# lazear/sage

Measured on AMD Instinct MI355X. Metric: spectra/sec (whole node), fragment-index search-and-score, human tryptic narrow search, higher is better.
Workload: dtype f32

## Files before the change

include/sage_hip.h:

```cpp
#ifndef SAGE_HIP_H
#define SAGE_HIP_H

#include <stddef.h>
#include <stdint.h>

#ifdef __cplusplus
extern "C" {
#endif

#define SAGE_HIP_ABI_VERSION 6

enum {
    SAGE_HIP_OK = 0,
    SAGE_HIP_ERR_INVALID = 1,
    SAGE_HIP_ERR_NO_DEVICE = 2,
    SAGE_HIP_ERR_HIP = 3,
    SAGE_HIP_ERR_UNSUPPORTED = 4,
    SAGE_HIP_ERR_OOM = 5,
    SAGE_HIP_ERR_INTERNAL = 6
};

enum { SAGE_TOL_PPM = 0, SAGE_TOL_PCT = 1, SAGE_TOL_DA = 2 };
typedef struct SageTolerance {
    int32_t kind;
// ... 161 lines not shown
    uint64_t* psm_off;
    uint8_t* kinds;
    int32_t* charges;
    int32_t* fragment_ordinals;
    float* intensities;
    float* mz_calculated;
    float* mz_experimental;
} SageFragments;
int sage_hip_annotate_resident(SageScorer* scorer, SageDeviceBatch* batch, const SageFeature* features,
                               const uint32_t* counts, SageFragments* out);

int sage_hip_quick_score_resident(SageScorer* scorer, SageDeviceBatch* batch, int prefilter_low_memory, uint8_t* keep);

typedef struct SageTiming {
    float prelim_ms;
    float rescore_ms;
    float total_ms;
    uint32_t n_launches;
    uint32_t n_wide;
    uint32_t arena_entries;
    uint32_t n_retry;
    float retry_ms;
    uint32_t n_tied;
    uint32_t n_ways;
} SageTiming;
int sage_hip_last_timing(const SageScorer* scorer, SageTiming* out);
int sage_hip_scorer_set_timing_interval(SageScorer* scorer, uint32_t every);

int sage_hip_host_alloc(uint64_t bytes, void** out);
void sage_hip_host_free(void* p);

int sage_hip_debug_phase_cycles(SageScorer* scorer, unsigned long long* out32);
int sage_hip_debug_prune_counters(SageScorer* scorer, unsigned long long* out4);

typedef struct SageRescoreInput {
    uint64_t n;
    const SageFeature* features;
    const float* aligned_rt;
    const float* delta_rt_model;
    const float* delta_ims_model;
    SageTolerance precursor_tol;
    const uint32_t* peptide_key;
    uint32_t n_peptide_keys;
    const uint32_t* protein_key;
    uint32_t n_protein_keys;
} SageRescoreInput;

typedef struct SageRescoreOutput {
    float* discriminant_score;
    float* posterior_error;
    float* spectrum_q;
    float* peptide_q;
    float* protein_q;
    uint32_t* order;
    uint64_t passing_spectrum;
    uint64_t passing_peptide;
    uint64_t passing_protein;
    int32_t lda_fitted;
    double coef[20];
    float device_ms;
} SageRescoreOutput;

int sage_hip_rescore(int device, const SageRescoreInput* in, SageRescoreOutput* out);

typedef struct SageRtInput {
    uint64_t n;
// ... 168 lines not shown
```

sage_amd/_lib.py:

```python
import ctypes as C
import os

import numpy as np

from . import build as _build

c_float_p = C.POINTER(C.c_float)
c_u8_p = C.POINTER(C.c_uint8)
c_u32_p = C.POINTER(C.c_uint32)
c_u64_p = C.POINTER(C.c_uint64)


class SageTolerance(C.Structure):
    _fields_ = [("kind", C.c_int32), ("lo", C.c_float), ("hi", C.c_float)]


class SageTheoretical(C.Structure):
    _fields_ = [("peptide_index", C.c_uint32), ("fragment_mz", C.c_float)]


class SageDbParams(C.Structure):
    _fields_ = [
        ("bucket_size", C.c_uint64),
        ("missed_cleavages", C.c_int32),
# ... 242 lines not shown
        "sage_hip_hostdb_build": (C.c_int, [C.c_char_p, C.POINTER(SageDbParams), C.POINTER(vp)]),
        "sage_hip_hostdb_free": (None, [vp]),
        "sage_hip_hostdb_view": (C.c_int, [vp, C.POINTER(SageDbView)]),
        "sage_hip_hostdb_peptide_string": (C.c_uint64, [vp, C.c_uint64, C.c_char_p, C.c_uint64]),
        "sage_hip_hostdb_peptide_proteins": (C.c_uint64, [vp, C.c_uint64, C.c_char_p, C.c_uint64]),
        "sage_hip_hostdb_peptide_info": (C.c_int, [vp, C.c_uint64, c_u32_p, c_u8_p]),
        "sage_hip_process_ms2": (C.c_uint64, [C.c_uint64, C.c_int, C.c_float, c_float_p, c_float_p, C.c_uint64,
                                              C.c_uint8, c_float_p, c_float_p, c_float_p]),
        "sage_hip_device_count": (C.c_int, []),
        "sage_hip_db_create": (C.c_int, [C.POINTER(SageDbView), C.c_int, C.POINTER(vp)]),
        "sage_hip_db_destroy": (None, [vp]),
        "sage_hip_db_device_bytes": (C.c_uint64, [vp]),
        "sage_hip_scorer_create": (C.c_int, [vp, C.POINTER(SageScorerParams), C.POINTER(vp)]),
        "sage_hip_scorer_destroy": (None, [vp]),
        "sage_hip_scorer_clone": (C.c_int, [vp, C.POINTER(vp)]),
        "sage_hip_score_batch": (C.c_int, [vp, C.POINTER(SageSpectrumBatch), vp, c_u32_p]),
        "sage_hip_batch_upload": (C.c_int, [vp, C.POINTER(SageSpectrumBatch), C.POINTER(vp)]),
        "sage_hip_batch_free": (None, [vp]),
        "sage_hip_batch_process_upload": (C.c_int, [vp, C.POINTER(SageRawBatch), C.c_uint64, C.c_int, C.c_float, C.c_uint32,
                                                    C.POINTER(vp), c_u32_p]),
        "sage_hip_batch_download": (C.c_int, [vp, c_u64_p, c_float_p, c_float_p, c_float_p]),
        "sage_hip_batch_upload_kinds": (C.c_int, [vp, C.POINTER(SageSpectrumBatch), c_u8_p, C.POINTER(vp)]),
        "sage_hip_batch_process_upload_kinds": (C.c_int, [vp, C.POINTER(SageRawBatch), c_u8_p, C.c_uint64, C.c_int, C.c_float,
                                                          C.c_uint32, C.POINTER(vp), c_u32_p]),
        "sage_hip_score_batch_kinds": (C.c_int, [vp, C.POINTER(SageSpectrumBatch), c_u8_p, vp, c_u32_p]),
        "sage_hip_score_resident": (C.c_int, [vp, vp, vp, c_u32_p]),
        "sage_hip_initial_hits": (C.c_int, [vp, vp, c_u64_p, C.c_uint32, c_u32_p, c_u64_p, c_u64_p]),
        "sage_hip_last_timing": (C.c_int, [vp, C.POINTER(SageTiming)]),
        "sage_hip_scorer_set_timing_interval": (C.c_int, [vp, C.c_uint32]),
        "sage_hip_annotate_resident": (C.c_int, [vp, vp, vp, c_u32_p, C.POINTER(SageFragments)]),
        "sage_hip_quick_score_resident": (C.c_int, [vp, vp, C.c_int, c_u8_p]),
        "sage_hip_debug_phase_cycles": (C.c_int, [vp, c_u64_p]),
        "sage_hip_debug_prune_counters": (C.c_int, [vp, c_u64_p]),
        "sage_hip_host_alloc": (C.c_int, [C.c_uint64, C.POINTER(vp)]),
        "sage_hip_host_free": (None, [vp]),
        "sage_hip_rescore": (C.c_int, [C.c_int, C.POINTER(SageRescoreInput), C.POINTER(SageRescoreOutput)]),
        "sage_hip_hostdb_competition_keys": (C.c_int, [vp, c_u32_p, C.c_uint64, c_u32_p, c_u32_p, c_u32_p, c_u32_p]),
        "sage_hip_predict_rt": (C.c_int, [C.c_int, C.POINTER(SageRtInput), C.POINTER(SageRtOutput)]),
        "sage_hip_hostdb_feature_peptides": (C.c_int, [vp, c_u32_p, C.c_uint64, c_u64_p, c_u8_p, c_float_p]),
        "sage_hip_mzml_read": (C.c_int, [C.c_char_p, C.c_uint32, C.c_int, C.POINTER(vp)]),
        "sage_hip_mzml_view": (C.c_int, [vp, C.POINTER(SageRawBatch)]),
        "sage_hip_mzml_check_searchable": (C.c_int, [vp]),
        "sage_hip_mzml_spectrum_id": (C.c_char_p, [vp, C.c_uint64]),
        "sage_hip_mzml_free": (None, [vp]),
        "sage_hip_mzml_read_sn": (C.c_int, [C.c_char_p, C.c_uint32, C.c_int, C.c_int, C.POINTER(vp)]),
        "sage_hip_mzml_ion_injection_time": (C.c_float, [vp, C.c_uint64]),
        "sage_hip_mzml_precursor_ref": (C.c_char_p, [vp, C.c_uint64]),
        "sage_hip_mgf_read": (C.c_int, [C.c_char_p, C.c_uint32, C.POINTER(vp)]),
        "sage_hip_mzml_isolation_kinds": (C.c_int, [vp, c_u8_p]),
        "sage_hip_mzml_charge_zero": (C.c_int, [vp, c_u8_p]),
        "sage_hip_parse_f32": (C.c_int, [C.c_char_p, C.c_uint64, c_float_p]),
        "sage_hip_tmt": (C.c_int, [C.c_int, C.POINTER(SageTmtInput), C.POINTER(SageTmtOutput)]),
        "sage_hip_write_tmt": (C.c_int, [C.c_char_p, C.POINTER(C.c_char_p), C.c_uint32, C.c_uint64, c_u32_p, C.POINTER(C.c_char_p),
                                         c_float_p, c_float_p, C.POINTER(C.c_char_p), C.c_uint32]),
        "sage_hip_write_results": (C.c_int, [C.c_char_p, C.c_int, vp, vp, C.c_uint64, c_u64_p, c_u64_p, C.POINTER(C.c_char_p),
                                             C.c_uint32, C.POINTER(C.c_char_p), C.POINTER(SagePostColumns)]),
        "sage_hip_lfq": (C.c_int, [C.c_int, C.POINTER(SageLfqInput), C.POINTER(SageLfqOutput)]),
        "sage_hip_lfq_im": (C.c_int, [C.c_int, C.POINTER(SageLfqInput), C.POINTER(SageLfqMobility), C.POINTER(SageLfqOutput)]),
        "sage_hip_mzml_mobility": (c_float_p, [vp]),
        "sage_hip_mzml_has_mobility": (C.c_int, [vp, c_u8_p]),
        "sage_hip_write_lfq": (C.c_int, [C.c_char_p, vp, C.POINTER(SageLfqOutput), c_u64_p, C.c_uint64, C.POINTER(C.c_char_p),
                                         C.c_uint32]),
        "sage_hip_fasta_num_targets": (C.c_int, [C.c_char_p, C.POINTER(SageDbParams), c_u64_p]),
        "sage_hip_prefilter_chunk_size": (C.c_int, [C.c_char_p, C.POINTER(SageDbParams), C.c_uint64, c_u64_p]),
        "sage_hip_hostdb_build_chunk": (C.c_int, [C.c_char_p, C.POINTER(SageDbParams), C.c_uint64, C.c_uint64, C.POINTER(vp)]),
        "sage_hip_hostdb_merge_kept": (C.c_int, [C.POINTER(vp), C.POINTER(c_u8_p), C.c_uint32, C.POINTER(SageDbParams),
                                                 C.POINTER(vp)]),
    }
    for name, (res, args) in sig.items():
        fn = getattr(lib, name)
        fn.restype = res
        fn.argtypes = args
    _lib = lib
    return lib


EXPORTED_SYMBOLS = [
    "sage_hip_last_error", "sage_hip_abi_version", "sage_hip_hostdb_build", "sage_hip_hostdb_free",
    "sage_hip_hostdb_view", "sage_hip_hostdb_peptide_string", "sage_hip_hostdb_peptide_proteins",
    "sage_hip_hostdb_peptide_info", "sage_hip_process_ms2", "sage_hip_device_count", "sage_hip_db_create", "sage_hip_db_destroy",
    "sage_hip_db_device_bytes", "sage_hip_scorer_create", "sage_hip_scorer_destroy", "sage_hip_scorer_clone", "sage_hip_score_batch",
    "sage_hip_batch_upload", "sage_hip_batch_free", "sage_hip_batch_process_upload", "sage_hip_batch_download", "sage_hip_score_resident", "sage_hip_initial_hits",
    "sage_hip_last_timing", "sage_hip_scorer_set_timing_interval", "sage_hip_annotate_resident", "sage_hip_quick_score_resident", "sage_hip_debug_phase_cycles", "sage_hip_debug_prune_counters", "sage_hip_host_alloc", "sage_hip_host_free",
    "sage_hip_rescore", "sage_hip_hostdb_competition_keys", "sage_hip_fasta_num_targets", "sage_hip_prefilter_chunk_size",
    "sage_hip_hostdb_build_chunk", "sage_hip_hostdb_merge_kept", "sage_hip_predict_rt", "sage_hip_hostdb_feature_peptides",
    "sage_hip_write_results", "sage_hip_mzml_read", "sage_hip_mzml_view", "sage_hip_mzml_check_searchable", "sage_hip_mzml_spectrum_id", "sage_hip_mzml_free",
    "sage_hip_lfq", "sage_hip_write_lfq", "sage_hip_mzml_read_sn", "sage_hip_mzml_ion_injection_time", "sage_hip_mzml_precursor_ref",
    "sage_hip_tmt", "sage_hip_write_tmt", "sage_hip_mgf_read", "sage_hip_mzml_isolation_kinds", "sage_hip_mzml_charge_zero",
    "sage_hip_parse_f32", "sage_hip_batch_upload_kinds", "sage_hip_batch_process_upload_kinds", "sage_hip_score_batch_kinds",
    "sage_hip_lfq_im", "sage_hip_mzml_mobility", "sage_hip_mzml_has_mobility",
]


def check(rc):
    if rc != 0:
        msg = load().sage_hip_last_error()
        raise SageHipError(f"libsage_hip status {rc}: {msg.decode() if msg else ''}")


def as_ptr(arr, ctype):
    return arr.ctypes.data_as(C.POINTER(ctype))
```

sage_amd/csrc/capi.hip:

```cpp
#include <hip/hip_runtime.h>
#include <algorithm>
#include <atomic>
#include <cmath>
#include <chrono>
#include <cstring>
#include <memory>
#include <future>
#include <mutex>
#include <string>
#include <vector>

#include "crlog.h"
#include "device_types.h"
#define HIP_FAILED(e, what) fail(status_of(e), std::string(what) + ": " + hipGetErrorString(e))
#include "hip_host.h"
#include "host_db.hpp"

using namespace sagehip;

namespace {

thread_local std::string g_last_error;

int fail(int code, const std::string& msg) {
// ... 2018 lines not shown
    if (rc != SAGE_HIP_OK) return rc;
    const uint32_t n = b->n, kmax = s->dev.kmax;
    std::vector<uint64_t> c((size_t)n * kmax);
    std::vector<uint32_t> tot((size_t)n * 2), st(n);
    HIP_TRY(hipMemcpy(c.data(), s->ws.cand.p, c.size() * 8, hipMemcpyDeviceToHost));
    HIP_TRY(hipMemcpy(len, s->ws.cand_len.p, (size_t)n * 4, hipMemcpyDeviceToHost));
    HIP_TRY(hipMemcpy(tot.data(), s->ws.totals.p, tot.size() * 4, hipMemcpyDeviceToHost));
    HIP_TRY(hipMemcpy(st.data(), s->ws.status.p, (size_t)n * 4, hipMemcpyDeviceToHost));
    for (uint32_t i = 0; i < n; i++) {
        if (st[i] != ST_OK && st[i] != ST_OK_ORDERED) return fail(SAGE_HIP_ERR_UNSUPPORTED, "spectrum " + std::to_string(i) + ": status " + std::to_string(st[i]));
        for (uint32_t j = 0; j < len[i]; j++) packed[(size_t)i * cap + j] = c[(size_t)i * kmax + j];
        if (matched_peaks) matched_peaks[i] = tot[2 * i];
        if (scored_candidates) scored_candidates[i] = tot[2 * i + 1];
    }
    return SAGE_HIP_OK;
}

int sage_hip_debug_phase_cycles(SageScorer* s, unsigned long long* out32) {
    if (!s || !out32) return fail(SAGE_HIP_ERR_INVALID, "null argument");
    if (!s->dbg.p) return fail(SAGE_HIP_ERR_INVALID, "set SAGE_HIP_PHASE_CLOCKS=1 before creating the scorer");
    std::vector<unsigned long long> all(4096 * 32);
    HIP_TRY(hipMemcpy(all.data(), s->dbg.p, all.size() * 8, hipMemcpyDeviceToHost));
    for (int k = 0; k < 32; k++) out32[k] = 0;
    for (size_t b = 0; b < 4096; b++)
        for (int k = 0; k < 32; k++) out32[k] += all[b * 32 + k];
    return SAGE_HIP_OK;
}

int sage_hip_debug_prune_counters(SageScorer* s, unsigned long long* out4) {
    if (!s || !out4) return fail(SAGE_HIP_ERR_INVALID, "null argument");
    if (!s->dbg.p) return fail(SAGE_HIP_ERR_INVALID, "set SAGE_HIP_PHASE_CLOCKS=1 before creating the scorer");
    std::vector<unsigned long long> all((size_t)DBG_BLOCKS * DBG_PRUNE_WORDS);
    HIP_TRY(hipMemcpy(all.data(), s->dbg.p + (size_t)DBG_BLOCKS * 32, all.size() * 8, hipMemcpyDeviceToHost));
    for (uint32_t k = 0; k < DBG_PRUNE_WORDS; k++) out4[k] = 0;
    for (size_t b = 0; b < DBG_BLOCKS; b++)
        for (uint32_t k = 0; k < DBG_PRUNE_WORDS; k++) out4[k] += all[b * DBG_PRUNE_WORDS + k];
    return SAGE_HIP_OK;
}

int sage_hip_host_alloc(uint64_t bytes, void** out) {
    if (!out) return fail(SAGE_HIP_ERR_INVALID, "null argument");
    HIP_TRY(hipHostMalloc(out, bytes ? bytes : 1, hipHostMallocDefault));
    if (void* d = device_view(*out)) {
        std::lock_guard<std::mutex> lock(g_blocks_mu);
        g_blocks.push_back(HostBlock{(const unsigned char*)*out, (unsigned char*)d, (size_t)(bytes ? bytes : 1)});
    }
    return SAGE_HIP_OK;
}
void sage_hip_host_free(void* p) {
    if (!p) return;
    {
        std::lock_guard<std::mutex> lock(g_blocks_mu);
        for (size_t i = 0; i < g_blocks.size(); i++)
            if (g_blocks[i].host == (const unsigned char*)p) {
                g_blocks.erase(g_blocks.begin() + (long)i);
                break;
            }
    }
    (void)hipHostFree(p);
}

int sage_hip_scorer_set_timing_interval(SageScorer* s, uint32_t every) {
    if (!s) return fail(SAGE_HIP_ERR_INVALID, "null argument");
    std::lock_guard<std::mutex> lock(s->mu);
    s->timing_every = every;
    s->timing_calls = 0;
    return SAGE_HIP_OK;
}

// ... 28 lines not shown
```

sage_amd/csrc/core.h:

```cpp
#pragma once
#include <stdint.h>

#if defined(__HIPCC__)
#define SAGE_HD __host__ __device__ __forceinline__
#else
#define SAGE_HD inline
#endif

namespace sagecore {

constexpr float PROTON = 1.0072764f;
constexpr float NEUTRON = 1.00335f;

struct Tol {
    int kind;
    float lo, hi;
};

SAGE_HD void tol_bounds(const Tol& t, float center, float& out_lo, float& out_hi) {
    if (t.kind == 0) {
        float dlo = center * t.lo / 1000000.0f;
        float dhi = center * t.hi / 1000000.0f;
        out_lo = center + dlo;
        out_hi = center + dhi;
// ... 477 lines not shown
    uint32_t x;
    asm("v_cvt_u32_f32 %0, %1" : "=v"(x) : "v"(f));
    return x;
#else
    const float f = ion * PBM_INV_W;
    return f >= 4294967296.0f ? 0xFFFFFFFFu : f > 0.0f ? (uint32_t)f : 0u;
#endif
}
SAGE_HD uint32_t pbm_bin_c1(uint32_t x) { return x & (PBM_BITS - 1u); }
SAGE_HD uint32_t pbm_bin_c2(uint32_t x) { return (x >> 1) & (PBM_BITS - 1u); }
SAGE_HD uint32_t pbm_bin_c3(uint32_t x) { return (uint32_t)(((uint64_t)x * 0xAAAAAAABull) >> 33) & (PBM_BITS - 1u); }
struct PbmReach {
    float a, b;
};
SAGE_HD PbmReach pbm_reach_of(const Tol& t) {
    const float tmax = __builtin_fmaxf(__builtin_fabsf(t.lo), __builtin_fabsf(t.hi));
    const float rel = t.kind == 0 ? tmax * 1.0e-6f : t.kind == 1 ? tmax * 1.0e-2f : 0.0f;
    PbmReach r{-1.0f, 0.0f};
    if (!(tmax == tmax) || !(tmax < 1.0e30f) || !(rel < 0.25f)) return r;
    r.a = (rel / (1.0f - rel)) * 1.0002f + (1.0f / 1048576.0f);
    r.b = (t.kind == 2 ? tmax * 1.0002f : 0.0f) + (1.0f / 1048576.0f);
    return r;
}
SAGE_HD bool pbm_peak_reach(const PbmReach& r, float m, float& D) {
    D = __builtin_fmaf(m, r.a, r.b);
    return r.a >= 0.0f && m >= 0.0f && m < 8388608.0f && D <= PBM_MAX_D;
}
SAGE_HD void pbm_peak_span(float m, float D, uint32_t& b0, uint32_t& b1) {
    const float f0 = (m - D) * PBM_INV_W, f1 = (m + D) * PBM_INV_W;
    b0 = f0 > 0.0f ? (uint32_t)f0 : 0u;
    b1 = f1 > 0.0f ? (uint32_t)f1 : 0u;
}

}
```

sage_amd/csrc/device_types.h:

```cpp
#pragma once
#include <stdint.h>

#include <string>

#include "../../include/sage_hip.h"
#include "core.h"

namespace sagehip {

struct DevDbView {
    const float* pep_mono;
    uint32_t np;
    const uint32_t* pep_lut;
    uint32_t pep_lut_bins;
    float pep_lut_inv_w;
    const SageTheoretical* pm_frag;
    const uint64_t* pm_off;
    const float* ions;
    const uint64_t* ion_off;
    const uint32_t* pep_info;
    const SageTheoretical* tm_frag;
    const uint32_t* tm_lut;
    uint32_t tile_shift;
    uint32_t n_tiles;
    uint32_t lut_stride;
    float lut_scale;
    const SageTheoretical* tm2_frag;
    const sagecore::LutWord* tm2_l1;
    const uint32_t* tm2_pos;
    uint32_t lut2_words;
    uint32_t tile2_shift;
    uint32_t n_tiles2;
    uint32_t lut2_stride;
    float lut2_scale;
    uint64_t nf;
    uint8_t ion_kinds[8];
    uint32_t n_kinds;
};

#ifndef SAGE_TM_LUT_TRANSPOSED
#define SAGE_TM_LUT_TRANSPOSED 0
#endif
#ifndef SAGE_TM_LUT_QUAD
#define SAGE_TM_LUT_QUAD 0
#endif
constexpr int TM_LUT_LAYOUT = SAGE_TM_LUT_QUAD != 0 ? 2 : SAGE_TM_LUT_TRANSPOSED != 0 ? 1 : 0;
constexpr bool TM_LUT_TRANSPOSED = TM_LUT_LAYOUT == 1;
__host__ __device__ inline uint32_t tm_lut_rows(uint32_t n_tiles) { return TM_LUT_LAYOUT == 2 ? (n_tiles + 3u) & ~3u : n_tiles; }
__host__ __device__ inline size_t tm_lut_index(uint32_t t, uint32_t c, uint32_t n_tiles, uint32_t lut_stride) {
    return TM_LUT_LAYOUT == 2 ? (((size_t)(t >> 2) * lut_stride + c) << 2) + (t & 3u)
           : TM_LUT_LAYOUT == 1 ? (size_t)c * n_tiles + t : (size_t)t * lut_stride + c;
}

constexpr uint32_t DBG_BLOCKS = 4096, DBG_PRUNE_WORDS = 4;
constexpr size_t DBG_TOTAL_WORDS = (size_t)DBG_BLOCKS * (32 + DBG_PRUNE_WORDS);

struct DevScorer {
    sagecore::Tol precursor_tol, fragment_tol;
    sagecore::PbmReach pbm_reach;
    uint32_t min_matched_peaks;
    int min_isotope_err, max_isotope_err;
    uint32_t min_precursor_charge, max_precursor_charge;
    uint32_t override_precursor_charge;
    int max_fragment_charge;
    uint32_t chimera;
    uint32_t report_psms;
    uint32_t wide_window;
    int score_type;
    uint32_t kmax;
    uint32_t big_path;
    uint32_t long_runs;
    uint32_t tol_mode;
    uint32_t list_cap;
    uint32_t wcap;
    uint32_t dbg_flags;
    uint32_t prune_min;
    uint32_t rescore_general;
    uint32_t xcd_chunk;
    uint32_t fast_log;
    uint32_t exact;
};

struct DevBatchView {
    uint32_t n;
    const uint32_t* n_dev;
    uint32_t spec_base;
    const uint64_t* peak_off;
// ... 160 lines not shown
```

sage_amd/csrc/kernels.hip:

```cpp
#include <hip/hip_runtime.h>

#include <type_traits>

#include "crlog.h"
#include "device_types.h"

using namespace sagecore;

namespace sagehip {

namespace {

constexpr uint32_t WAVE = 64;
constexpr uint32_t FAST_TIE_WORDS = PBM_WORDS + PLUT_BINS;
constexpr uint32_t CNT_ROW_HEADER = 4;
#ifndef SAGE_PROBE_PER_LANE
#define SAGE_PROBE_PER_LANE 2
#endif
constexpr uint32_t PROBE_BATCH_WORDS = SAGE_PROBE_PER_LANE * 64;
constexpr uint32_t PROBE_TCS_WORDS = PROBE_BATCH_WORDS <= 64 ? 64 : PROBE_BATCH_WORDS <= 128 ? 128 : PROBE_BATCH_WORDS <= 256 ? 256 : 512;
constexpr uint32_t PROBE_TABLE_WORDS = 4 * PROBE_BATCH_WORDS + PROBE_TCS_WORDS;

enum { DBG_PRUNE_CAND = 0, DBG_PRUNE_ITEMS = 1, DBG_PRUNE_EARLY = 2, DBG_PRUNE_MIXED = 3 };
enum { DBG_NARROW_LUT = 26, DBG_NARROW_CELLS = 27, DBG_RESCORE = 28, DBG_TILE_LUT = 29, DBG_TILE_CELLS = 30, DBG_TILE_CAND = 31 };
struct PhaseClock {
    unsigned long long* slot;
    long long t;
    __device__ __forceinline__ void bytes(int which, unsigned long long n) {
        if (slot) atomicAdd(&slot[which - row_base], n);
    }
    int row_base;
    unsigned long long* prune;
    uint32_t pruned_here;
    __device__ __forceinline__ void pruned(uint64_t lanes, uint32_t items) {
        if (slot && lanes) {
            pruned_here += (uint32_t)__popcll(lanes);
            if ((threadIdx.x & 63u) == 0) {
                atomicAdd(&prune[DBG_PRUNE_CAND], (unsigned long long)__popcll(lanes));
                atomicAdd(&prune[DBG_PRUNE_ITEMS], (unsigned long long)items);
            }
        }
    }
    __device__ __forceinline__ void prune_outcome(bool left_early, bool any_pass) {
        if (slot && (threadIdx.x & 63u) == 0) {
            if (left_early) atomicAdd(&prune[DBG_PRUNE_EARLY], 1ull);
            else if (any_pass && pruned_here) atomicAdd(&prune[DBG_PRUNE_MIXED], 1ull);
        }
        pruned_here = 0;
    }
    __device__ __forceinline__ void start(unsigned long long* dbg, uint32_t blk, uint32_t kernel) {
        slot = dbg ? dbg + (size_t)(blk % DBG_BLOCKS) * 32 + kernel * 8 : nullptr;
        row_base = (int)kernel * 8;
        prune = dbg ? dbg + (size_t)DBG_BLOCKS * 32 + (size_t)(blk % DBG_BLOCKS) * DBG_PRUNE_WORDS : nullptr;
        pruned_here = 0;
        if (slot) t = clock64();
    }
    __device__ __forceinline__ void mark(int phase) {
        if (slot) {
            const long long n = clock64();
            if ((threadIdx.x & 63u) == 0) atomicAdd(&slot[phase], (unsigned long long)(n - t));
            t = n;
        }
    }
    __device__ __forceinline__ void rebase(uint32_t kernel) {
        if (slot) slot += (int)kernel * 8 - row_base;
        row_base = (int)kernel * 8;
    }
};

struct NoClock {
    static constexpr unsigned long long* slot = nullptr;
    __device__ __forceinline__ void bytes(int, unsigned long long) {}
    __device__ __forceinline__ void pruned(uint64_t, uint32_t) {}
    __device__ __forceinline__ void prune_outcome(bool, bool) {}
    __device__ __forceinline__ void start(unsigned long long*, uint32_t, uint32_t) {}
    __device__ __forceinline__ void mark(int) {}
    __device__ __forceinline__ void rebase(uint32_t) {}
};

__device__ __forceinline__ uint32_t lane_id() { return threadIdx.x & 63u; }

#ifndef SAGE_STAGGER_NS
#define SAGE_STAGGER_NS 0
#endif
__device__ __forceinline__ void staggered_start(uint32_t blk) {
    if (SAGE_STAGGER_NS > 0 && blk >= 1024u && blk < 5u * 1024u) {
        const uint32_t slot = blk / 1024u;
        const long long until = (long long)__builtin_amdgcn_s_memtime() + (long long)slot * (SAGE_STAGGER_NS * 2);
        while ((long long)__builtin_amdgcn_s_memtime() < until) __builtin_amdgcn_s_sleep(32);
    }
}

constexpr uint32_t N_XCD = 8;
__device__ __forceinline__ uint32_t xcd_position_fwd(uint32_t b, uint32_t n, uint32_t chunk) {
    if (chunk == 0) return b;
    const uint32_t group = N_XCD * chunk;
    if (b >= n / group * group) return b;
    const uint32_t x = b % N_XCD, i = b / N_XCD;
    return ((i / chunk) * N_XCD + x) * chunk + i % chunk;
}
__device__ __forceinline__ uint32_t xcd_position(uint32_t b, uint32_t n, uint32_t chunk) {
    const uint32_t p = xcd_position_fwd(b, n, chunk & 0x7FFFFFFFu);
    return (chunk & 0x80000000u) ? n - 1 - p : p;
}

__device__ __forceinline__ uint32_t fresh_zero() {
    uint32_t z;
// ... 2442 lines not shown
    if (a.longest_b != b.longest_b) return a.longest_b > b.longest_b;
    if (a.longest_y != b.longest_y) return a.longest_y > b.longest_y;
    if (!(a.hyperscore == b.hyperscore)) return a.hyperscore > b.hyperscore;
    if (!(a.ppm_difference == b.ppm_difference)) return a.ppm_difference > b.ppm_difference;
    if (a.charge != b.charge) return a.charge > b.charge;
    return a.iso > b.iso;
}

struct RescoreLds {
    uint32_t* pbm;
    uint32_t* plut;
    double* s_sorted;
    long long* s_key;
    QuickKey* qkeys;
    uint32_t* hdr;
    uint2* meta;
    float* pm;
    float* pi;
    uint8_t* rm;
    uint8_t* rm2;
    uint32_t* stage;
};
constexpr uint32_t FEATURE_WORDS = sizeof(SageFeature) / 4;
static_assert(sizeof(SageFeature) == 120, "Feature records leave LDS as 30 dwords");
__host__ __device__ inline uint32_t stage_records(const DevScorer& sc) { return sc.big_path ? 0u : sc.chimera ? 1u : sc.report_psms; }
__host__ __device__ inline size_t rescore_scratch_bytes(bool quick) {
    static_assert(PBM_WORDS * 4 >= 64 * 8 + 64 * 8, "s_sorted + s_key fit the bitmap");
    static_assert(FAST_TIE_WORDS == PBM_WORDS + PLUT_BINS, "the fast-tie replay stages its counts over pbm + plut, contiguous below");
    return (size_t)PBM_WORDS * 4 + PLUT_BINS * 4 + (quick ? 64 * sizeof(QuickKey) : 0);
}
constexpr uint32_t RESCORE_HDR_WORDS = 8;
enum RescoreHdr { HDR_TIC = 0, HDR_MZP = 1, HDR_RT = 2, HDR_IMS = 3, HDR_FILE = 4, HDR_MATCHED = 5, HDR_SCORED = 6 };
constexpr size_t RESCORE_HEAD_BYTES = RESCORE_HDR_WORDS * 4 + 64 * sizeof(uint2);
__host__ __device__ inline size_t rescore_fixed_bytes(const DevScorer& sc, const DevBatchView& b) {
    const size_t n = RESCORE_HEAD_BYTES + (size_t)b.pcap * 8 + (((size_t)b.pcap * 2 + 7) & ~(size_t)7) + (size_t)stage_records(sc) * sizeof(SageFeature);
    return (n + 15) & ~(size_t)15;
}
__device__ __forceinline__ RescoreLds carve_rescore(unsigned char* scratch, unsigned char* fixed, const DevBatchView& b) {
    RescoreLds l;
    l.pbm = (uint32_t*)scratch;
    l.plut = l.pbm + PBM_WORDS;
    l.s_sorted = (double*)l.pbm;
    l.s_key = (long long*)(l.s_sorted + 64);
    l.qkeys = (QuickKey*)(l.plut + PLUT_BINS);
    l.hdr = (uint32_t*)fixed;
    l.meta = (uint2*)(fixed + RESCORE_HDR_WORDS * 4);
    l.pm = (float*)(fixed + RESCORE_HEAD_BYTES);
    l.pi = l.pm + b.pcap;
    l.rm = (uint8_t*)(l.pi + b.pcap);
    l.rm2 = l.rm + b.pcap;
    l.stage = (uint32_t*)(fixed + RESCORE_HEAD_BYTES + (size_t)b.pcap * 8 + (((size_t)b.pcap * 2 + 7) & ~(size_t)7));
    return l;
}

__device__ __forceinline__ uint32_t lane_run(uint32_t v, uint32_t src_lane) { return (uint32_t)__builtin_amdgcn_readlane((int)v, (int)src_lane); }
__device__ __forceinline__ uint64_t lane_run(uint64_t v, uint32_t src_lane) { return lane_value(v, src_lane); }
#ifndef SAGE_DENSE_HITS
#define SAGE_DENSE_HITS 1
#endif
constexpr uint32_t DENSE_CAP = 384;
static_assert(DENSE_CAP % 64 == 0 && DENSE_CAP * 10 + DENSE_CAP / 8 <= PBM_WORDS * 4, "the dense work list fits the bitmap");
template <class PC, bool LONG = false, bool FAST = false>
__device__ __forceinline__ void score_candidates(const DevDbView& db, const DevScorer& sc, const uint32_t* pbm, const uint32_t* plut,
                                                 const float* pm, const float* pi, const uint32_t P, const float inv_w,
                                                 const bool valid, const uint64_t ion_base, const uint32_t lm1, const uint32_t nfz,
                                                 const bool any_fz2, const bool any_fz3, const uint32_t nterm_mask, const bool sym_tol,
                                                 Score& s, PC& pc, const bool have_first = false, const float first0 = 0.f,
                                                 const float first1 = 0.f, const float first2 = 0.f, const float first3 = 0.f,
                                                 const bool dense_ok = false) {
    const uint32_t lane = lane_id();
    typedef typename std::conditional<LONG, uint64_t, uint32_t>::type RunReg;
    constexpr bool DENSE = !LONG;
    RunReg b_run = 0, y_run = 0;
    uint32_t mm = 0;
    const bool scored = valid && lm1 && nfz;
    const float* __restrict__ my = db.ions + ion_base;
    const uint32_t nions = scored ? db.n_kinds * lm1 : 0u;
    for (uint32_t j0 = 0; __ballot(j0 < nions) != 0ull; j0 += 64u) {
        const bool act = j0 < nions;
        const uint32_t n_here = !act ? 0u : nions - j0 < 64u ? nions - j0 : 64u;
        uint64_t m1 = 0, m2 = 0, m3 = 0;
        if (act) {
            const float* __restrict__ q = my + j0;
            float n0, n1, n2, n3;
            if (have_first && j0 == 0) { n0 = first0; n1 = first1; n2 = first2; n3 = first3; }
            else { n0 = q[0]; n1 = q[1]; n2 = q[2]; n3 = q[3]; }
            for (uint32_t r = 0; r < n_here; r += 4) {
                const float i0 = n0, i1 = n1, i2 = n2, i3 = n3;
                n0 = q[r + 4]; n1 = q[r + 5]; n2 = q[r + 6]; n3 = q[r + 7];
                const uint32_t x0 = pbm_index(i0), x1 = pbm_index(i1), x2 = pbm_index(i2), x3 = pbm_index(i3);
                const uint32_t t1 = pbm_bit(x0) | (pbm_bit(x1) << 1) | (pbm_bit(x2) << 2) | (pbm_bit(x3) << 3);
                m1 |= (uint64_t)t1 << r;
                if (any_fz2) {
                    const uint32_t t2 = pbm_bit(x0 >> 1) | (pbm_bit(x1 >> 1) << 1) | (pbm_bit(x2 >> 1) << 2) | (pbm_bit(x3 >> 1) << 3);
                    m2 |= (uint64_t)t2 << r;
                }
                if (any_fz3) {
                    const uint32_t t3 = pbm_bit(__umulhi(x0, 0xAAAAAAABu) >> 1) | (pbm_bit(__umulhi(x1, 0xAAAAAAABu) >> 1) << 1) |
                                        (pbm_bit(__umulhi(x2, 0xAAAAAAABu) >> 1) << 2) | (pbm_bit(__umulhi(x3, 0xAAAAAAABu) >> 1) << 3);
                    m3 |= (uint64_t)t3 << r;
                }
            }
            const uint64_t in_chunk = n_here >= 64u ? ~0ull : (1ull << n_here) - 1ull;
            m1 &= in_chunk;
            m2 = nfz >= 2 ? m2 & in_chunk : 0ull;
            m3 = nfz >= 3 ? m3 & in_chunk : 0ull;
            if (nfz > 3) m1 = m2 = m3 = in_chunk;
        }
        pc.mark(6);
        uint32_t hc = act && nfz <= 3 ? (uint32_t)(__popcll(m1) + __popcll(m2) + __popcll(m3)) : 0u;
        {
            const bool drop = hc != 0u && j0 + 64u >= nions && (mm & 0xFFFFu) + (mm >> 16) + hc < sc.prune_min;
            if (pc.slot) pc.pruned(__ballot(drop), wave_sum(drop ? hc : 0u));
            if (drop) {
                m1 = m2 = m3 = 0ull;
                hc = 0u;
            }
        }
        uint64_t bigs = (sc.dbg_flags & 32u) ? 0ull : __ballot(hc > COOP_MIN_HITS);
        if ((uint32_t)__popcll(bigs) > COOP_MAX_LANES && !(sc.dbg_flags & 64u)) bigs = 0ull;
        while (bigs) {
            const uint32_t L = (uint32_t)__ffsll((long long)bigs) - 1;
            bigs &= bigs - 1;
            const uint64_t M1 = lane_value(m1, L), M2 = lane_value(m2, L), M3 = lane_value(m3, L);
            const uint64_t base_L = lane_value((uint64_t)ion_base, L);
            const uint32_t lm1_L = (uint32_t)__builtin_amdgcn_readlane((int)lm1, (int)L);
            const bool on1 = (M1 >> lane) & 1ull, on2 = (M2 >> lane) & 1ull, on3 = (M3 >> lane) & 1ull;
            float it1 = 0.f, it2 = 0.f, it3 = 0.f, tm1 = 0.f, tm2 = 0.f, tm3 = 0.f;
            bool ok1 = false, ok2 = false, ok3 = false;
            if (on1 || on2 || on3) {
                const float ionv = db.ions[base_L + j0 + lane];
#define SAGE_COOP_LOOKUP(C, ON, OK, IT, TM)                                                              \
    if (ON) {                                                                                            \
        const float mz = fragment_mz<FAST>(ionv, (C));                                                   \
        float flo, fhi;                                                                                  \
// ... 333 lines not shown
        float first0 = 0.f, first1 = 0.f, first2 = 0.f, first3 = 0.f;
        if (round == 0 && valid) {
            const uint32_t plen = pep_rec & 0xFFFFu;
            lm1 = db.n_kinds && plen ? plen - 1u : 0u;
            R.meta[lane] = make_uint2(pep_rec, __float_as_uint(pep_mass));
            if (SAGE_ION_PREFETCH && lm1 && nfz) {
                const float* __restrict__ q = db.ions + ion_base;
                first0 = q[0]; first1 = q[1]; first2 = q[2]; first3 = q[3];
            }
        }
        if (round == 0) build_peak_bitmap(pbm, pm, P, sc.pbm_reach);
        lds_sync();
        if (round == 0) {
        if (pc.slot) {
            const uint32_t ion_bytes = wave_sum(valid ? 4u * db.n_kinds * lm1 + 24u : 0u);
            const uint32_t ncand = (uint32_t)__popcll(__ballot(mine != PRESCORE_EMPTY));
            if (lane == 0) pc.bytes(DBG_RESCORE, 8ull * P + 8ull * ncand + ion_bytes);
            const uint32_t items = wave_sum(SAGE_N_ITEMS);
            uint32_t longest = SAGE_N_ITEMS;
            for (int o = 32; o; o >>= 1) { const uint32_t v = (uint32_t)__shfl_xor((int)longest, o, 64); longest = v > longest ? v : longest; }
            const uint32_t nvalid = (uint32_t)__popcll(__ballot(valid));
            (void)items; (void)longest; (void)nvalid;
        }
        }
        Score s;
        s.peptide = 0;
        s.precursor_charge = 0;
        s.isotope_error = 0;
        s.matched_b = s.matched_y = 0;
        s.summed_b = s.summed_y = 0.0f;
        s.ppm_difference = 0.0f;
        s.longest_b = s.longest_y = 0;
        pc.mark(5);
        score_candidates<PC, false, FAST>(db, sc, pbm, plut, pm, pi, P, inv_w, valid, ion_base, lm1, nfz, any_fz2, any_fz3, nterm_mask, sym_tol,
                                          s, pc, SAGE_ION_PREFETCH && round == 0, first0, first1, first2, first3, !CHIMERA || !sc.chimera);
        pc.mark(1);
        LateArgs<KA> la(db, sc, b, w, lnfact_table, lnfact_n, out, out_count);
        la.refresh();
        {
            const uint32_t prune_min = la.prune_min();
            const uint64_t can_pass = __ballot(valid && s.matched_b + s.matched_y >= prune_min);
            const bool leave = prune_min != 0u && can_pass == 0ull;
            pc.prune_outcome(leave, can_pass != 0ull);
            if (leave) {
                if (ACC && keep) return true;
                break;
            }
        }
        const double lambda = (double)R.hdr[HDR_MATCHED] / (double)R.hdr[HDR_SCORED];
        double h = 0.0;
        bool pass = false;
        bool ln_undecided;
        const double ln_i = cr_log_pair<ACC>(hyperscore_arg(s), lambda, round == 0, ((__ballot(valid) >> 63) & 1ull) == 0ull, ln_lambda, ln_undecided);
        if (__builtin_expect(!ACC && __ballot(ln_undecided && (valid || round == 0)) != 0ull, 0)) {
            if (queue_on_tie && lane == 0) {
                la.status()[spec] = ST_RETRY;
                la.retry()[atomicAdd(la.counters() + CTR_RETRY, 1u)] = spec;
                la.out_count()[spec] = 0;
            }
            return false;
        }
        if (valid) {
            s.ppm_difference /= s.summed_b + s.summed_y;
            h = hyperscore_dev(la.score_type(), s, ln_i, la.lnfact_table(), la.lnfact_n());
            pass = (s.matched_b + s.matched_y) >= la.min_matched_peaks();
        }
        const uint32_t report_psms = la.report_psms();
// ... 944 lines not shown
```

Before: 139.1 million.

## Redistribute candidate ion filtering across the wave via a flat LDS work list

After: 141.3 million, median of 6. 1.02x the previous value.

```diff
diff --git a/include/sage_hip.h b/include/sage_hip.h
--- a/include/sage_hip.h
+++ b/include/sage_hip.h
@@ -217,6 +217,7 @@
 
 int sage_hip_debug_phase_cycles(SageScorer* scorer, unsigned long long* out32);
 int sage_hip_debug_prune_counters(SageScorer* scorer, unsigned long long* out4);
+int sage_hip_debug_filter_counters(SageScorer* scorer, unsigned long long* out4);
 
 typedef struct SageRescoreInput {
     uint64_t n;
diff --git a/sage_amd/_lib.py b/sage_amd/_lib.py
--- a/sage_amd/_lib.py
+++ b/sage_amd/_lib.py
@@ -298,6 +298,7 @@
         "sage_hip_quick_score_resident": (C.c_int, [vp, vp, C.c_int, c_u8_p]),
         "sage_hip_debug_phase_cycles": (C.c_int, [vp, c_u64_p]),
         "sage_hip_debug_prune_counters": (C.c_int, [vp, c_u64_p]),
+        "sage_hip_debug_filter_counters": (C.c_int, [vp, c_u64_p]),
         "sage_hip_host_alloc": (C.c_int, [C.c_uint64, C.POINTER(vp)]),
         "sage_hip_host_free": (None, [vp]),
         "sage_hip_rescore": (C.c_int, [C.c_int, C.POINTER(SageRescoreInput), C.POINTER(SageRescoreOutput)]),
@@ -347,7 +348,7 @@
     "sage_hip_hostdb_peptide_info", "sage_hip_process_ms2", "sage_hip_device_count", "sage_hip_db_create", "sage_hip_db_destroy",
     "sage_hip_db_device_bytes", "sage_hip_scorer_create", "sage_hip_scorer_destroy", "sage_hip_scorer_clone", "sage_hip_score_batch",
     "sage_hip_batch_upload", "sage_hip_batch_free", "sage_hip_batch_process_upload", "sage_hip_batch_download", "sage_hip_score_resident", "sage_hip_initial_hits",
-    "sage_hip_last_timing", "sage_hip_scorer_set_timing_interval", "sage_hip_annotate_resident", "sage_hip_quick_score_resident", "sage_hip_debug_phase_cycles", "sage_hip_debug_prune_counters", "sage_hip_host_alloc", "sage_hip_host_free",
+    "sage_hip_last_timing", "sage_hip_scorer_set_timing_interval", "sage_hip_annotate_resident", "sage_hip_quick_score_resident", "sage_hip_debug_phase_cycles", "sage_hip_debug_prune_counters", "sage_hip_debug_filter_counters", "sage_hip_host_alloc", "sage_hip_host_free",
     "sage_hip_rescore", "sage_hip_hostdb_competition_keys", "sage_hip_fasta_num_targets", "sage_hip_prefilter_chunk_size",
     "sage_hip_hostdb_build_chunk", "sage_hip_hostdb_merge_kept", "sage_hip_predict_rt", "sage_hip_hostdb_feature_peptides",
     "sage_hip_write_results", "sage_hip_mzml_read", "sage_hip_mzml_view", "sage_hip_mzml_check_searchable", "sage_hip_mzml_spectrum_id", "sage_hip_mzml_free",
diff --git a/sage_amd/csrc/capi.hip b/sage_amd/csrc/capi.hip
--- a/sage_amd/csrc/capi.hip
+++ b/sage_amd/csrc/capi.hip
@@ -2074,9 +2074,19 @@
     if (!s->dbg.p) return fail(SAGE_HIP_ERR_INVALID, "set SAGE_HIP_PHASE_CLOCKS=1 before creating the scorer");
     std::vector<unsigned long long> all((size_t)DBG_BLOCKS * DBG_PRUNE_WORDS);
     HIP_TRY(hipMemcpy(all.data(), s->dbg.p + (size_t)DBG_BLOCKS * 32, all.size() * 8, hipMemcpyDeviceToHost));
-    for (uint32_t k = 0; k < DBG_PRUNE_WORDS; k++) out4[k] = 0;
+    for (uint32_t k = 0; k < 4; k++) out4[k] = 0;
     for (size_t b = 0; b < DBG_BLOCKS; b++)
-        for (uint32_t k = 0; k < DBG_PRUNE_WORDS; k++) out4[k] += all[b * DBG_PRUNE_WORDS + k];
+        for (uint32_t k = 0; k < 4; k++) out4[k] += all[b * DBG_PRUNE_WORDS + k];
+    return SAGE_HIP_OK;
+}
+int sage_hip_debug_filter_counters(SageScorer* s, unsigned long long* out4) {
+    if (!s || !out4) return fail(SAGE_HIP_ERR_INVALID, "null argument");
+    if (!s->dbg.p) return fail(SAGE_HIP_ERR_INVALID, "set SAGE_HIP_PHASE_CLOCKS=1 before creating the scorer");
+    std::vector<unsigned long long> all((size_t)DBG_BLOCKS * DBG_PRUNE_WORDS);
+    HIP_TRY(hipMemcpy(all.data(), s->dbg.p + (size_t)DBG_BLOCKS * 32, all.size() * 8, hipMemcpyDeviceToHost));
+    for (uint32_t k = 0; k < 4; k++) out4[k] = 0;
+    for (size_t b = 0; b < DBG_BLOCKS; b++)
+        for (uint32_t k = 0; k < 4; k++) out4[k] += all[b * DBG_PRUNE_WORDS + 4 + k];
     return SAGE_HIP_OK;
 }
 
diff --git a/sage_amd/csrc/core.h b/sage_amd/csrc/core.h
--- a/sage_amd/csrc/core.h
+++ b/sage_amd/csrc/core.h
@@ -533,4 +533,25 @@
     b1 = f1 > 0.0f ? (uint32_t)f1 : 0u;
 }
 
-}
+SAGE_HD uint32_t flat_octets(uint32_t n_here) { return (n_here + 7u) >> 3; }
+SAGE_HD uint32_t flat_item_k(uint32_t t, uint32_t owner_start) { return t - owner_start; }
+SAGE_HD uint64_t flat_item_base(uint64_t chunk_at, uint32_t owner_start) { return chunk_at - 8ull * owner_start; }
+SAGE_HD uint64_t flat_item_ion(uint64_t item_base, uint32_t t) { return item_base + 8ull * t; }
+SAGE_HD uint32_t flat_stride(uint32_t total) { return (total + 3u) & ~3u; }
+SAGE_HD uint32_t flat_area_bytes(uint32_t total, uint32_t ncharges) { return flat_stride(total) * ncharges + 12u; }
+#ifndef SAGE_FLAT_MARGIN
+#define SAGE_FLAT_MARGIN 1
+#endif
+constexpr uint32_t FLAT_MARGIN = SAGE_FLAT_MARGIN;
+SAGE_HD uint32_t flat_route_bar(uint32_t total) { return (total + 63u) / 64u + FLAT_MARGIN; }
+SAGE_HD bool flat_route_wins(uint32_t total, uint32_t longest) { return total != 0u && longest > flat_route_bar(total); }
+SAGE_HD uint32_t flat_mask_word(uint32_t lo, uint32_t hi, uint32_t start) {
+#if defined(__HIP_DEVICE_COMPILE__)
+    return __builtin_amdgcn_alignbyte(hi, lo, start & 3u);
+#else
+    const uint32_t sh = (start & 3u) * 8u;
+    return sh ? (lo >> sh) | (hi << (32u - sh)) : lo;
+#endif
+}
+
+}
diff --git a/sage_amd/csrc/device_types.h b/sage_amd/csrc/device_types.h
--- a/sage_amd/csrc/device_types.h
+++ b/sage_amd/csrc/device_types.h
@@ -52,7 +52,7 @@
            : TM_LUT_LAYOUT == 1 ? (size_t)c * n_tiles + t : (size_t)t * lut_stride + c;
 }
 
-constexpr uint32_t DBG_BLOCKS = 4096, DBG_PRUNE_WORDS = 4;
+constexpr uint32_t DBG_BLOCKS = 4096, DBG_PRUNE_WORDS = 8;
 constexpr size_t DBG_TOTAL_WORDS = (size_t)DBG_BLOCKS * (32 + DBG_PRUNE_WORDS);
 
 struct DevScorer {
diff --git a/sage_amd/csrc/kernels.hip b/sage_amd/csrc/kernels.hip
--- a/sage_amd/csrc/kernels.hip
+++ b/sage_amd/csrc/kernels.hip
@@ -22,6 +22,7 @@
 constexpr uint32_t PROBE_TABLE_WORDS = 4 * PROBE_BATCH_WORDS + PROBE_TCS_WORDS;
 
 enum { DBG_PRUNE_CAND = 0, DBG_PRUNE_ITEMS = 1, DBG_PRUNE_EARLY = 2, DBG_PRUNE_MIXED = 3 };
+enum { DBG_FILTER_FLAT_CHUNKS = 4, DBG_FILTER_FLAT_TRIPS = 5, DBG_FILTER_FLAT_WOULD = 6, DBG_FILTER_LANE_TRIPS = 7 };
 enum { DBG_NARROW_LUT = 26, DBG_NARROW_CELLS = 27, DBG_RESCORE = 28, DBG_TILE_LUT = 29, DBG_TILE_CELLS = 30, DBG_TILE_CAND = 31 };
 struct PhaseClock {
     unsigned long long* slot;
@@ -41,6 +42,17 @@
             }
         }
     }
+    __device__ __forceinline__ void filter_trips(bool flat, uint32_t flat_trips, uint32_t lane_trips) {
+        if (slot && (threadIdx.x & 63u) == 0) {
+            if (flat) {
+                atomicAdd(&prune[DBG_FILTER_FLAT_CHUNKS], 1ull);
+                atomicAdd(&prune[DBG_FILTER_FLAT_TRIPS], (unsigned long long)flat_trips);
+                atomicAdd(&prune[DBG_FILTER_FLAT_WOULD], (unsigned long long)lane_trips);
+            } else {
+                atomicAdd(&prune[DBG_FILTER_LANE_TRIPS], (unsigned long long)lane_trips);
+            }
+        }
+    }
     __device__ __forceinline__ void prune_outcome(bool left_early, bool any_pass) {
         if (slot && (threadIdx.x & 63u) == 0) {
             if (left_early) atomicAdd(&prune[DBG_PRUNE_EARLY], 1ull);
@@ -73,6 +85,7 @@
     __device__ __forceinline__ void bytes(int, unsigned long long) {}
     __device__ __forceinline__ void pruned(uint64_t, uint32_t) {}
     __device__ __forceinline__ void prune_outcome(bool, bool) {}
+    __device__ __forceinline__ void filter_trips(bool, uint32_t, uint32_t) {}
     __device__ __forceinline__ void start(unsigned long long*, uint32_t, uint32_t) {}
     __device__ __forceinline__ void mark(int) {}
     __device__ __forceinline__ void rebase(uint32_t) {}
@@ -2581,10 +2594,13 @@
 constexpr uint32_t RESCORE_HDR_WORDS = 8;
 enum RescoreHdr { HDR_TIC = 0, HDR_MZP = 1, HDR_RT = 2, HDR_IMS = 3, HDR_FILE = 4, HDR_MATCHED = 5, HDR_SCORED = 6 };
 constexpr size_t RESCORE_HEAD_BYTES = RESCORE_HDR_WORDS * 4 + 64 * sizeof(uint2);
+constexpr uint32_t FLAT_EXTRA_BYTES = 384;
+__host__ __device__ inline uint32_t rescore_flat_bytes(uint32_t pcap) { return ((pcap * 2u + 7u) & ~7u) + FLAT_EXTRA_BYTES; }
 __host__ __device__ inline size_t rescore_fixed_bytes(const DevScorer& sc, const DevBatchView& b) {
-    const size_t n = RESCORE_HEAD_BYTES + (size_t)b.pcap * 8 + (((size_t)b.pcap * 2 + 7) & ~(size_t)7) + (size_t)stage_records(sc) * sizeof(SageFeature);
+    const size_t n = RESCORE_HEAD_BYTES + (size_t)b.pcap * 8 + rescore_flat_bytes(b.pcap) + (size_t)stage_records(sc) * sizeof(SageFeature);
     return (n + 15) & ~(size_t)15;
 }
+__device__ __forceinline__ uint8_t* rescore_flat_area(const float* pm, const float* pi) { return (uint8_t*)(pi + (pi - pm)); }
 __device__ __forceinline__ RescoreLds carve_rescore(unsigned char* scratch, unsigned char* fixed, const DevBatchView& b) {
     RescoreLds l;
     l.pbm = (uint32_t*)scratch;
@@ -2596,9 +2612,9 @@
     l.meta = (uint2*)(fixed + RESCORE_HDR_WORDS * 4);
     l.pm = (float*)(fixed + RESCORE_HEAD_BYTES);
     l.pi = l.pm + b.pcap;
-    l.rm = (uint8_t*)(l.pi + b.pcap);
+    l.rm = rescore_flat_area(l.pm, l.pi);
     l.rm2 = l.rm + b.pcap;
-    l.stage = (uint32_t*)(fixed + RESCORE_HEAD_BYTES + (size_t)b.pcap * 8 + (((size_t)b.pcap * 2 + 7) & ~(size_t)7));
+    l.stage = (uint32_t*)(fixed + RESCORE_HEAD_BYTES + (size_t)b.pcap * 8 + rescore_flat_bytes(b.pcap));
     return l;
 }
 
@@ -2609,7 +2625,10 @@
 #endif
 constexpr uint32_t DENSE_CAP = 384;
 static_assert(DENSE_CAP % 64 == 0 && DENSE_CAP * 10 + DENSE_CAP / 8 <= PBM_WORDS * 4, "the dense work list fits the bitmap");
-template <class PC, bool LONG = false, bool FAST = false>
+#ifndef SAGE_FLAT_GENERAL
+#define SAGE_FLAT_GENERAL 0
+#endif
+template <class PC, bool LONG = false, bool FAST = false, bool FLAT = !LONG>
 __device__ __forceinline__ void score_candidates(const DevDbView& db, const DevScorer& sc, const uint32_t* pbm, const uint32_t* plut,
                                                  const float* pm, const float* pi, const uint32_t P, const float inv_w,
                                                  const bool valid, const uint64_t ion_base, const uint32_t lm1, const uint32_t nfz,
@@ -2617,6 +2636,8 @@
                                                  Score& s, PC& pc, const bool have_first = false, const float first0 = 0.f,
                                                  const float first1 = 0.f, const float first2 = 0.f, const float first3 = 0.f,
                                                  const bool dense_ok = false) {
+    static_assert(!(FLAT && LONG), "the flat route's worker offsets and tags are those of the one-register instances");
+    const bool flat_ok = FLAT && !(sc.dbg_flags & 8192u);
     const uint32_t lane = lane_id();
     typedef typename std::conditional<LONG, uint64_t, uint32_t>::type RunReg;
     constexpr bool DENSE = !LONG;
@@ -2629,7 +2650,79 @@
         const bool act = j0 < nions;
         const uint32_t n_here = !act ? 0u : nions - j0 < 64u ? nions - j0 : 64u;
         uint64_t m1 = 0, m2 = 0, m3 = 0;
-        if (act) {
+        bool flat = false;
+        uint32_t flat_trips = 0;
+        if (flat_ok) {
+            uint8_t* const flat_area = rescore_flat_area(pm, pi);
+            const uint32_t flat_cap = rescore_flat_bytes((uint32_t)(pi - pm));
+            const uint32_t cnt = act && nfz <= 3u ? flat_octets(n_here) : 0u;
+            const uint32_t incl = wave_incl_scan_dpp(cnt), start = incl - cnt;
+            const uint32_t T = (uint32_t)__builtin_amdgcn_readlane((int)incl, 63);
+            const uint32_t stride = flat_stride(T);
+            if (T != 0u && flat_area_bytes(T, 1u + (any_fz2 ? 1u : 0u) + (any_fz3 ? 1u : 0u)) <= flat_cap &&
+                (__ballot(cnt > flat_route_bar(T)) != 0ull || (sc.dbg_flags & 16384u))) {
+                flat = true;
+                uint8_t* const a1 = flat_area;
+                uint8_t* const a2 = a1 + stride;
+                uint8_t* const a3 = a2 + (any_fz2 ? stride : 0u);
+                for (uint32_t k = 0; __ballot(k < cnt) != 0ull; k++)
+                    if (k < cnt) a1[start + k] = (uint8_t)lane;
+                lds_sync();
+                const uint64_t ion_at = flat_item_base(ion_base + j0, start);
+                for (uint32_t base = 0; base < T; base += WAVE) {
+                    const uint32_t t = base + lane;
+                    const bool on = t < T;
+                    const uint32_t src = (on ? (uint32_t)a1[t] : 0u) << 2;
+                    const uint64_t ib = ((uint64_t)(uint32_t)__builtin_amdgcn_ds_bpermute((int)src, (int)(uint32_t)(ion_at >> 32)) << 32) |
+                                        (uint32_t)__builtin_amdgcn_ds_bpermute((int)src, (int)(uint32_t)ion_at);
+                    if (on) {
+                        const float* __restrict__ q = db.ions + flat_item_ion(ib, t);
+                        const float i0 = q[0], i1 = q[1], i2 = q[2], i3 = q[3], i4 = q[4], i5 = q[5], i6 = q[6], i7 = q[7];
+                        const uint32_t x0 = pbm_index(i0), x1 = pbm_index(i1), x2 = pbm_index(i2), x3 = pbm_index(i3);
+                        const uint32_t x4 = pbm_index(i4), x5 = pbm_index(i5), x6 = pbm_index(i6), x7 = pbm_index(i7);
+#define SAGE_FLAT_BYTE(F)                                                                                             \
+    (uint8_t)(pbm_bit(F(x0)) | (pbm_bit(F(x1)) << 1) | (pbm_bit(F(x2)) << 2) | (pbm_bit(F(x3)) << 3) | (pbm_bit(F(x4)) << 4) | \
+              (pbm_bit(F(x5)) << 5) | (pbm_bit(F(x6)) << 6) | (pbm_bit(F(x7)) << 7))
+#define SAGE_FLAT_C1(X) (X)
+#define SAGE_FLAT_C2(X) ((X) >> 1)
+#define SAGE_FLAT_C3(X) (__umulhi((X), 0xAAAAAAABu) >> 1)
+                        a1[t] = SAGE_FLAT_BYTE(SAGE_FLAT_C1);
+                        if (any_fz2) a2[t] = SAGE_FLAT_BYTE(SAGE_FLAT_C2);
+                        if (any_fz3) a3[t] = SAGE_FLAT_BYTE(SAGE_FLAT_C3);
+#undef SAGE_FLAT_C3
+#undef SAGE_FLAT_C2
+#undef SAGE_FLAT_C1
+#undef SAGE_FLAT_BYTE
+                    }
+                }
+                lds_sync();
+                if (cnt != 0u) {
+                    const uint32_t at = start & ~3u;
+                    {
+                        const uint32_t* const wp = (const uint32_t*)(a1 + at);
+                        const uint32_t w0 = wp[0], w1 = wp[1], w2 = wp[2];
+                        m1 = (uint64_t)flat_mask_word(w0, w1, start) | ((uint64_t)flat_mask_word(w1, w2, start) << 32);
+                    }
+                    if (any_fz2 && nfz >= 2u) {
+                        const uint32_t* const wp = (const uint32_t*)(a2 + at);
+                        const uint32_t w0 = wp[0], w1 = wp[1], w2 = wp[2];
+                        m2 = (uint64_t)flat_mask_word(w0, w1, start) | ((uint64_t)flat_mask_word(w1, w2, start) << 32);
+                    }
+                    if (any_fz3 && nfz >= 3u) {
+                        const uint32_t* const wp = (const uint32_t*)(a3 + at);
+                        const uint32_t w0 = wp[0], w1 = wp[1], w2 = wp[2];
+                        m3 = (uint64_t)flat_mask_word(w0, w1, start) | ((uint64_t)flat_mask_word(w1, w2, start) << 32);
+                    }
+                }
+            }
+            flat_trips = (T + 63u) / 64u;
+        }
+        if (pc.slot) {
+            uint32_t would = act ? (n_here + 3u) >> 2 : 0u;
+            for (int o = 32; o; o >>= 1) { const uint32_t v = (uint32_t)__shfl_xor((int)would, o, 64); would = v > would ? v : would; }
+            pc.filter_trips(flat, flat_trips, would);
+        }
+        if (act && !flat) {
             const float* __restrict__ q = my + j0;
             float n0, n1, n2, n3;
             if (have_first && j0 == 0) { n0 = first0; n1 = first1; n2 = first2; n3 = first3; }
@@ -2650,6 +2743,8 @@
                     m3 |= (uint64_t)t3 << r;
                 }
             }
+        }
+        if (act) {
             const uint64_t in_chunk = n_here >= 64u ? ~0ull : (1ull << n_here) - 1ull;
             m1 &= in_chunk;
             m2 = nfz >= 2 ? m2 & in_chunk : 0ull;
@@ -3049,7 +3144,7 @@
         s.ppm_difference = 0.0f;
         s.longest_b = s.longest_y = 0;
         pc.mark(5);
-        score_candidates<PC, false, FAST>(db, sc, pbm, plut, pm, pi, P, inv_w, valid, ion_base, lm1, nfz, any_fz2, any_fz3, nterm_mask, sym_tol,
+        score_candidates<PC, false, FAST, SAGE_FLAT_GENERAL || !CHIMERA>(db, sc, pbm, plut, pm, pi, P, inv_w, valid, ion_base, lm1, nfz, any_fz2, any_fz3, nterm_mask, sym_tol,
                                           s, pc, SAGE_ION_PREFETCH && round == 0, first0, first1, first2, first3, !CHIMERA || !sc.chimera);
         pc.mark(1);
         LateArgs<KA> la(db, sc, b, w, lnfact_table, lnfact_n, out, out_count);
```
